# gaspardol/MonteCarloPredictiveCoding

Hardware: AMD Instinct MI355X
Metric: Langevin inference steps/sec (whole node), MNIST MCPC 784-256-256-30, batch 6000 (higher is better)
Workload: dtype f32

## Files before the change

### include/mcpc.h

```cpp
#ifndef MCPC_H
#define MCPC_H

#include <stdint.h>

#ifdef __cplusplus
extern "C" {
#endif

#define MCPC_ABI_VERSION 4
#define MCPC_MAX_LATENT 6

#define MCPC_OK 0
#define MCPC_EINVAL (-1)
#define MCPC_EHIP (-2)
#define MCPC_ENOMEM (-3)
#define MCPC_ESTATE (-4)

#define MCPC_ACT_IDENTITY 0
#define MCPC_ACT_RELU 1
#define MCPC_ACT_TANH 2

#define MCPC_LOSS_NONE 0
#define MCPC_LOSS_GAUSSIAN 1
#define MCPC_LOSS_BERNOULLI 2
// ... 66 lines not shown
const char* mcpc_last_error(void);
int mcpc_create(const mcpc_net_desc* desc, mcpc_engine** out);
int mcpc_destroy(mcpc_engine* e);

int mcpc_bind_params(mcpc_engine* e, int j, const float* W, const float* bias);
int mcpc_params_changed(mcpc_engine* e, void* stream);

int mcpc_bind_inputs(mcpc_engine* e, const float* inputs, void* stream);
int mcpc_bind_target(mcpc_engine* e, const float* target, void* stream);

int mcpc_load_state(mcpc_engine* e, const float* const* x, void* stream);
int mcpc_store_state(mcpc_engine* e, float* const* x, void* stream);

int mcpc_store_adam_state(mcpc_engine* e, float* const* m, float* const* v, void* stream);

int mcpc_run(mcpc_engine* e, const mcpc_run_desc* run, void* stream);

int mcpc_read_param_grads(mcpc_engine* e, int j, float* dW, float* db, float scale, int accumulate, void* stream);
int mcpc_read_param_grads_flat(mcpc_engine* e, float* flat, int64_t n_floats, float scale, void* stream);
int64_t mcpc_param_count(const mcpc_engine* e);

#define MCPC_COMM_ID_BYTES 128
int mcpc_comm_unique_id(void* id_out);
int mcpc_comm_init(mcpc_engine* e, int n_ranks, int rank, const void* id);
int mcpc_allreduce_grads(mcpc_engine* e, float* flat, int64_t n_floats, void* stream);
int mcpc_comm_destroy(mcpc_engine* e);

int mcpc_philox_normals(int device, uint64_t seed, uint64_t step, int layer, uint64_t chain_base,
                        int batch, int n_units, float* out, int raw, void* stream);

#define MCPC_MOM_IDENTITY 0
#define MCPC_MOM_SIGMOID  1

int mcpc_moments_accumulate(int device, const float* rec, int64_t row_elems, int32_t first, int32_t stride, int32_t n,
                            int32_t transform, double* sum, double* sumsq, int accumulate, void* stream);

int mcpc_sync_check(mcpc_engine* e, void* stream);

int mcpc_query(const mcpc_engine* e, int32_t* lds_bytes, int32_t* chains_per_wg, int32_t* n_workgroups,
               int32_t* spill_slots);
const char* mcpc_step_kernel_name(const mcpc_engine* e);
const char* mcpc_last_step_kernel_name(const mcpc_engine* e);
const char* mcpc_last_flush_plan(const mcpc_engine* e, int j);

int mcpc_set_profiling(mcpc_engine* e, int enable);
int mcpc_last_step_kernel_ms(mcpc_engine* e, float* ms, int32_t* n_launches, int64_t* n_steps);
int mcpc_last_shader_clock_ghz(mcpc_engine* e, float* ghz);

int mcpc_debug_poison_lds(int device, uint32_t word, void* stream);

int mcpc_debug_lw_jobs(int32_t n_latent, const int32_t* sizes, int32_t n_out, int32_t* fwd, int32_t* bwd, int32_t cap,
                       int32_t* n_fwd, int32_t* n_bwd, int32_t* tile);

#ifdef __cplusplus
}
#endif
#endif
```

### montecarlopredictivecoding_amd/_lib.py

```python
import ctypes as C
import os

MAX_LATENT = 6
COMM_ID_BYTES = 128
ENERGY_COLS = MAX_LATENT + 2
ABI_VERSION = 4

ACT_IDENTITY, ACT_RELU, ACT_TANH = 0, 1, 2
LOSS_NONE, LOSS_GAUSSIAN, LOSS_BERNOULLI = 0, 1, 2
XOPT_SGD, XOPT_ADAM = 0, 1
NOISE_NONE, NOISE_PHILOX, NOISE_EXTERNAL = 0, 1, 2
ENERGY_NONE, ENERGY_LAST, ENERGY_ALL = 0, 1, 2
MOM_IDENTITY, MOM_SIGMOID = 0, 1

LIB_PATH = os.environ.get("MCPC_LIB") or os.path.join(os.path.dirname(os.path.abspath(__file__)), "libmcpc.so")


class MCPCLibraryError(RuntimeError):
    pass


class MCPCError(RuntimeError):

    def __init__(self, code, message):
# ... 25 lines not shown
        ("beta1", C.c_double), ("beta2", C.c_double), ("eps", C.c_double),
        ("update_x", C.c_int32),
        ("noise_mode", C.c_int32), ("noise_var", C.c_double),
        ("seed", C.c_uint64), ("step_base", C.c_uint64), ("chain_base", C.c_uint64),
        ("ext_noise", C.c_void_p * MAX_LATENT),
        ("acc_begin", C.c_int32), ("acc_end", C.c_int32), ("acc_reset", C.c_int32),
        ("energy_mode", C.c_int32),
        ("energies_out", C.c_void_p),
        ("rec_begin", C.c_int32), ("rec_stride", C.c_int32), ("rec_count", C.c_int32),
        ("rec_x", C.c_void_p * MAX_LATENT),
        ("rec_out", C.c_void_p),
        ("xgrad", C.c_void_p * MAX_LATENT),
    ]


SYMBOLS = {
    "mcpc_abi_version": (C.c_int, []),
    "mcpc_build_info": (C.c_char_p, []),
    "mcpc_last_error": (C.c_char_p, []),
    "mcpc_create": (C.c_int, [C.POINTER(NetDesc), C.POINTER(C.c_void_p)]),
    "mcpc_destroy": (C.c_int, [C.c_void_p]),
    "mcpc_bind_params": (C.c_int, [C.c_void_p, C.c_int, C.c_void_p, C.c_void_p]),
    "mcpc_params_changed": (C.c_int, [C.c_void_p, C.c_void_p]),
    "mcpc_bind_inputs": (C.c_int, [C.c_void_p, C.c_void_p, C.c_void_p]),
    "mcpc_bind_target": (C.c_int, [C.c_void_p, C.c_void_p, C.c_void_p]),
    "mcpc_load_state": (C.c_int, [C.c_void_p, C.POINTER(C.c_void_p), C.c_void_p]),
    "mcpc_store_state": (C.c_int, [C.c_void_p, C.POINTER(C.c_void_p), C.c_void_p]),
    "mcpc_store_adam_state": (C.c_int, [C.c_void_p, C.POINTER(C.c_void_p), C.POINTER(C.c_void_p), C.c_void_p]),
    "mcpc_run": (C.c_int, [C.c_void_p, C.POINTER(RunDesc), C.c_void_p]),
    "mcpc_read_param_grads": (C.c_int, [C.c_void_p, C.c_int, C.c_void_p, C.c_void_p, C.c_float, C.c_int, C.c_void_p]),
    "mcpc_read_param_grads_flat": (C.c_int, [C.c_void_p, C.c_void_p, C.c_int64, C.c_float, C.c_void_p]),
    "mcpc_param_count": (C.c_int64, [C.c_void_p]),
    "mcpc_comm_unique_id": (C.c_int, [C.c_void_p]),
    "mcpc_comm_init": (C.c_int, [C.c_void_p, C.c_int, C.c_int, C.c_void_p]),
    "mcpc_allreduce_grads": (C.c_int, [C.c_void_p, C.c_void_p, C.c_int64, C.c_void_p]),
    "mcpc_comm_destroy": (C.c_int, [C.c_void_p]),
    "mcpc_philox_normals": (C.c_int, [C.c_int, C.c_uint64, C.c_uint64, C.c_int, C.c_uint64, C.c_int, C.c_int,
                                      C.c_void_p, C.c_int, C.c_void_p]),
    "mcpc_moments_accumulate": (C.c_int, [C.c_int, C.c_void_p, C.c_int64, C.c_int32, C.c_int32, C.c_int32, C.c_int32,
                                          C.c_void_p, C.c_void_p, C.c_int, C.c_void_p]),
    "mcpc_query": (C.c_int, [C.c_void_p, C.POINTER(C.c_int32), C.POINTER(C.c_int32), C.POINTER(C.c_int32),
                             C.POINTER(C.c_int32)]),
    "mcpc_step_kernel_name": (C.c_char_p, [C.c_void_p]),
    "mcpc_last_step_kernel_name": (C.c_char_p, [C.c_void_p]),
    "mcpc_last_flush_plan": (C.c_char_p, [C.c_void_p, C.c_int]),
    "mcpc_sync_check": (C.c_int, [C.c_void_p, C.c_void_p]),
    "mcpc_set_profiling": (C.c_int, [C.c_void_p, C.c_int]),
    "mcpc_last_step_kernel_ms": (C.c_int, [C.c_void_p, C.POINTER(C.c_float), C.POINTER(C.c_int32),
                                           C.POINTER(C.c_int64)]),
    "mcpc_last_shader_clock_ghz": (C.c_int, [C.c_void_p, C.POINTER(C.c_float)]),
    "mcpc_debug_poison_lds": (C.c_int, [C.c_int, C.c_uint32, C.c_void_p]),
    "mcpc_debug_lw_jobs": (C.c_int, [C.c_int32, C.POINTER(C.c_int32), C.c_int32, C.POINTER(C.c_int32), C.POINTER(C.c_int32), C.c_int32,
                                     C.POINTER(C.c_int32), C.POINTER(C.c_int32), C.POINTER(C.c_int32)]),
}

_lib = None


def load():
    global _lib
    if _lib is not None:
        return _lib
    if not os.path.exists(LIB_PATH):
        raise MCPCLibraryError(
            f"{LIB_PATH} not found: build it with `python -c 'import __graft_entry__ as g; g.build()'` "
            f"or `make -C montecarlopredictivecoding_amd/csrc`. There is no fallback path.")
    import torch
    try:
        lib = C.CDLL(LIB_PATH)
    except OSError as exc:
        raise MCPCLibraryError(f"could not load {LIB_PATH}: {exc}") from exc
    for name, (res, args) in SYMBOLS.items():
        try:
            fn = getattr(lib, name)
        except AttributeError as exc:
            raise MCPCLibraryError(f"{LIB_PATH} does not export {name}") from exc
        fn.restype = res
        fn.argtypes = args
    v = lib.mcpc_abi_version()
    if v != ABI_VERSION:
        raise MCPCLibraryError(f"libmcpc ABI {v} != binding ABI {ABI_VERSION}: rebuild the library")
    info = parse_build_info(lib.mcpc_build_info().decode("utf-8", "replace"))
    if info.get("exp") != "0" and os.environ.get("MCPC_ALLOW_EXP") != "1":
        raise MCPCLibraryError(f"{LIB_PATH} is a timing-experiment build ({info.get('flags')}): it computes wrong results on purpose. "
                               "Set MCPC_ALLOW_EXP=1 to load it for a timing A/B; unset MCPC_LIB to load the product.")
    _lib = lib
    return lib


def parse_build_info(line: str) -> dict:
    head, _, flags = line.partition(" flags=[")
    out = {"flags": flags[:-1] if flags.endswith("]") else flags}
    for word in head.split()[1:]:
        key, _, val = word.partition("=")
        out[key] = val
    return out


def build_info() -> dict:
    info = parse_build_info(load().mcpc_build_info().decode("utf-8", "replace"))
    info["path"] = LIB_PATH
    return info


def csrc_sha(root=None) -> str:
    import glob
# ... 15 lines not shown
```

### montecarlopredictivecoding_amd/csrc/mcpc_api.hip

```cpp
#include <hip/hip_runtime.h>
#include <dlfcn.h>
#include <rccl/rccl.h>

#include <algorithm>
#include <cmath>
#include <cstdarg>
#include <cstdio>
#include <cstdlib>
#include <cstring>
#include <string>
#include <vector>

#include "mcpc_build.h"
#include "mcpc_kernels.h"
#include "mcpc_moments.h"

using namespace mcpc;

namespace {

thread_local std::string g_err;

int fail(int code, const char* fmt, ...) {
    char buf[1024];
// ... 4 lines not shown
    g_err = buf;
    return code;
}

#define HIP_TRY(expr)                                                                            \
    do {                                                                                         \
        hipError_t _e = (expr);                                                                  \
        if (_e != hipSuccess) return fail(MCPC_EHIP, "%s failed: %s (%s:%d)", #expr, hipGetErrorString(_e), __FILE__, __LINE__); \
    } while (0)

inline int pad16(int n) { return (n + 15) / 16 * 16; }
inline int kblocks(int k_pad) { return (k_pad + kKB - 1) / kKB; }
inline int grid_for(size_t n, int block = 256) { return (int)std::min<size_t>((n + block - 1) / block, 4096); }
inline bool heb_wide(int et, int at) { return et >= 8 && at % 8 == 0 && (at <= 16 || at % 16 == 0); }
inline bool heb_narrow_in(int et, int at) { return !heb_wide(et, at) && et == 16 && (at == 1 || at == 2 || at == 4); }

struct Lin {
    const float* W = nullptr;
    const float* bias = nullptr;
    bool bound = false;
    int n_out = 0, n_in = 0, out_pad = 0, in_pad = 0;
    float* Wf = nullptr;
    float* Wb = nullptr;
    float* bias_pad = nullptr;
    float* G = nullptr;
    float* Gb = nullptr;
    int g_ld = 0;
    bool spill_tm = false;
    size_t slab_off = 0;
    size_t slab_floats = 0;
};

constexpr int kMaxRingParts = 8;
struct Knobs {
    int ws = -1;
    int wide = 0;
    int no_overlap = 0;
    int slot_cap = 384;
    int spill_gb = 0;
    int cu_slack = 0;
    int flush_streams = 2;
    int flush_tail = 0;
    int ring_parts = 3;
    int dw_ksplit = 0;
    int ws_prio = 0;
    int stagger = 0;
    int no_lean = 0;
    int no_ybits = 0;
    int overlay16 = 0;
    int no_xl = 0;
    int rr = 1;
    int rr_qmax = 100;
    int heb171 = 0;
    int heb_fp32 = 0;
    int u_row = 5000;
    int u_gemm0 = 1200;
    int u_kb = 200;
    int u_kbt = 68;
    int u_eh = 3000, u_eb = 1300, u_ef = 500;
};

int parse_tuning(const char* str, Knobs& k) {
    if (!str) return 0;
    std::string s(str);
    size_t pos = 0;
    while (pos < s.size()) {
        size_t end = s.find_first_of(",;", pos);
        if (end == std::string::npos) end = s.size();
        std::string item = s.substr(pos, end - pos);
        pos = end + 1;
        while (!item.empty() && item.front() == ' ') item.erase(item.begin());
        while (!item.empty() && item.back() == ' ') item.pop_back();
        if (item.empty()) continue;
        const size_t eq = item.find('=');
        const std::string key = item.substr(0, eq);
        const int val = eq == std::string::npos ? 1 : atoi(item.c_str() + eq + 1);
        struct { const char* name; int* dst; } table[] = {
            {"ws", &k.ws}, {"wide", &k.wide}, {"no_overlap", &k.no_overlap},
            {"slot_cap", &k.slot_cap}, {"spill_gb", &k.spill_gb}, {"cu_slack", &k.cu_slack}, {"ring_parts", &k.ring_parts}, {"flush_tail", &k.flush_tail}, {"flush_streams", &k.flush_streams}, {"dw_ksplit", &k.dw_ksplit},
            {"ws_prio", &k.ws_prio}, {"stagger", &k.stagger}, {"no_lean", &k.no_lean}, {"no_ybits", &k.no_ybits}, {"overlay16", &k.overlay16}, {"heb_fp32", &k.heb_fp32}, {"heb171", &k.heb171}, {"rr", &k.rr}, {"rr_qmax", &k.rr_qmax}, {"no_xl", &k.no_xl},
            {"u_row", &k.u_row}, {"u_gemm0", &k.u_gemm0}, {"u_kb", &k.u_kb}, {"u_kbt", &k.u_kbt}, {"u_eh", &k.u_eh}, {"u_eb", &k.u_eb}, {"u_ef", &k.u_ef}};
        bool found = false;
        for (auto& t : table)
            if (key == t.name) { *t.dst = val; found = true; }
        if (!found) return fail(MCPC_EINVAL, "unknown tuning key '%s' in mcpc_net_desc::tuning", key.c_str());
    }
    if (k.ws != -1 && k.ws != 0 && k.ws != 2 && k.ws != 3 && k.ws != 4)
        return fail(MCPC_EINVAL, "tuning ws=%d: 0 (barrier kernel), 2 (in-place kernel), 3 (unified-wave kernel) or 4 (layer-wise kernels)", k.ws);
    if (k.ws == 4) {
        const Knobs dflt;
        const struct { const char* name; bool set; } lds_only[] = {
            {"no_lean", k.no_lean != 0}, {"no_xl", k.no_xl != 0}, {"overlay16", k.overlay16 != 0}, {"rr", k.rr != dflt.rr},
            {"u_row", k.u_row != dflt.u_row}, {"u_gemm0", k.u_gemm0 != dflt.u_gemm0}, {"u_kb", k.u_kb != dflt.u_kb}, {"u_kbt", k.u_kbt != dflt.u_kbt},
            {"u_eh", k.u_eh != dflt.u_eh}, {"u_eb", k.u_eb != dflt.u_eb}, {"u_ef", k.u_ef != dflt.u_ef}};
        for (auto& t : lds_only)
            if (t.set) return fail(MCPC_EINVAL, "tuning ws=4 (layer-wise kernels) together with %s, a knob of the LDS-resident kernels", t.name);
    }
    if (k.slot_cap < 2) k.slot_cap = 2;
    if (k.cu_slack < 0) k.cu_slack = 0;
    if (k.ring_parts < 2 || k.ring_parts > kMaxRingParts) return fail(MCPC_EINVAL, "tuning ring_parts=%d: 2..%d", k.ring_parts, kMaxRingParts);
    return 0;
}

}

static const char* const kLwName = "mcpc::mcpc_lw_fwd_kernel + mcpc::mcpc_lw_bwd_kernel";

struct UPlan {
    bool ok = false;
    bool on = false;
    bool prefer = false;
    int lds_a[kMaxLatent]{}, lds_e[kMaxLatent]{}, lds_eo = 0, lds_red = 0, lds_ws_sync = 0, lds_zero = 0, lds_spillmax = 0, lds_rowexp = 0;
    int lds_x[kMaxLatent]{}, lds_bias[kMaxLatent]{}, lds_hbias = 0, lds_yw = 0, lds_bytes = 0;
    KPhase* phases = nullptr;
    int n_phases = 0;
};

struct mcpc_engine {
    mcpc_net_desc d{};
    Knobs knobs;
    ncclComm_t comm = nullptr;
    int comm_ranks = 0;
    int L = 0, Bpad = 0, nwg = 0, has_head = 0;
    int nwg_live = 0;
    static constexpr int ct = 16;
    int nw = kWaves;
    int ws = 0;
    int ws2_chunk = 0, ws2_ring = 0;
    bool ws2_overlay = true;
    int lds_ws_sync = 0;
    int npad[kMaxLatent]{};
    int out_pad = 0;
    Lin lin[kMaxLatent + 1];
    float* x[kMaxLatent]{};
    float* m[kMaxLatent]{};
    float* v[kMaxLatent]{};
    float* e0sum = nullptr;
    float* mu1 = nullptr;
    float* ypad = nullptr;
    float* ytile = nullptr;
    uint32_t* ybits = nullptr;
    int* y_binary = nullptr;
    int ywords = 0;
    bool target_bound = false;
    const float* inputs = nullptr;
    int slots = 0, half_slots = 0;
    hipStream_t aux = nullptr;
    hipEvent_t ev_steps[kMaxRingParts] = {}, ev_flush[kMaxRingParts] = {};
    hipStream_t spacer = nullptr;
    hipStream_t aux3 = nullptr;
// ... 1105 lines not shown
    const int nlin = e->L + (e->has_head ? 1 : 0);
    const int max_rows = e->half_slots * e->Bpad;
    size_t total = 0;
    for (int j = 1; j < nlin; ++j) {
        Lin& ln = e->lin[j];
        const HebPlan h = plan_hebbian(e, ln.out_pad, ln.in_pad, max_rows);
        ln.slab_off = total;
        ln.slab_floats = (size_t)h.ksplit_cap * ((size_t)ln.out_pad * ln.in_pad + ln.out_pad);
        total += ln.slab_floats;
    }
    if (!e->slab && (rc = dmalloc(e->slab, total))) return rc;
    e->slab_floats = total;
    e->spill_ready = true;
    return 0;
}

static inline int spill_id_a_host(int l) { return l; }
int flush_spill(mcpc_engine* e, int n_slots, int slot0, hipStream_t stream, int part) {
    const unsigned* const smax = e->spillmax + (size_t)part * kSpillTensors;
    const int rows = n_slots * e->Bpad;
    const int nlin = e->L + (e->has_head ? 1 : 0);
    ReduceJobs jobs{};
    unsigned max_blocks = 1;
    hipStream_t const main_stream = stream;
    const bool two = e->aux3 != nullptr && stream == e->aux;
    double load[2] = {0.0, 0.0};
    if (two) { HIP_TRY(hipEventRecord(e->ev_fork, main_stream)); HIP_TRY(hipStreamWaitEvent(e->aux3, e->ev_fork, 0)); }
    auto next_stream = [&](double cost) {
        const int k = (two && load[1] < load[0]) ? 1 : 0;
        load[k] += cost;
        return k ? e->aux3 : main_stream;
    };
    for (int j = 1; j < nlin; ++j) {
        Lin& ln = e->lin[j];
        const int ne = ln.out_pad, na = ln.in_pad;
        const float* E = (j < e->L ? e->spill_e[j] : e->spill_eo) + (size_t)slot0 * e->Bpad * ne;
        const float* A = e->spill_a[j - 1] + (size_t)slot0 * e->Bpad * na;
        const HebPlan h = plan_hebbian(e, ne, na, rows);
        std::string plan;
        auto name_launch = [&](const char* kern, int te, int ra, bool sw, int n_mt, int n_nt) {
            char buf[64];
            snprintf(buf, sizeof buf, "%s%s<%d,%d%s>x%d", plan.empty() ? "" : "+", kern, te, ra, sw ? ",T" : "", n_mt);
            plan += buf;
            if (n_nt > 1) plan += "*" + std::to_string(n_nt);
        };
        const char* const heb_name = e->knobs.heb_fp32 ? "heb" : "heb7";
        const int e_id = j < e->L ? kMaxLatent + j : kSpillIdEo;
        float* slab = e->slab + ln.slab_off;
        float* slab_b = slab + (size_t)h.ksplit * ne * na;
        if ((size_t)h.ksplit * ((size_t)ne * na + ne) > ln.slab_floats)
            return fail(MCPC_ESTATE, "internal: Hebbian slabs of Linear %d (%d splits) exceed their allocation", j, h.ksplit);
        if (h.swapped) {
            stream = next_stream((double)ne * na);
            HebArgs a{A, E, slab, slab_b, rows, na, ne, h.rps, 1, 1, h.ksplit, 0, smax + spill_id_a_host(j - 1), smax + e_id};
            name_launch(heb_name, h.te[0], 2, true, 1, 1);
            int rc = 0;
            if (!e->knobs.heb_fp32) {
                if (h.te[0] == 1) rc = launch_heb7<1, 2, true>(a, stream);
                else if (h.te[0] == 2) rc = launch_heb7<2, 2, true>(a, stream);
                else rc = launch_heb7<4, 2, true>(a, stream);
            } else
            if (h.te[0] == 1) rc = launch_heb<1, 2, true>(a, stream);
            else if (h.te[0] == 2) rc = launch_heb<2, 2, true>(a, stream);
            else rc = launch_heb<4, 2, true>(a, stream);
            if (rc) return rc;
        } else if (h.tiled) {
            int col = 0;
            for (int part = 0; part < 2; ++part) {
                if (h.n_mt[part] == 0) continue;
                HebArgs a{E, A, slab, slab_b, rows, ne, na, h.rps, h.n_mt[part], h.n_nt, h.ksplit, col, smax + e_id, smax + spill_id_a_host(j - 1)};
                stream = next_stream((double)h.n_mt[part] * h.te[part] * 16 * na);
                int rc = 0;
                const int te = h.te[part];
                const bool resplit = te == 17 && h.ra == 2 && !e->knobs.heb_fp32 && e->knobs.heb171;
                if (!resplit) name_launch(heb_name, te, h.ra, false, h.n_mt[part], h.n_nt);
                if (!e->knobs.heb_fp32) {
                    if (te == 17 && h.ra == 2 && !e->knobs.heb171) rc = launch_heb7<17, 2>(a, stream);
                    else if (te == 17 && h.ra == 2) {
                        HebArgs a1 = a;
                        a1.n_nt = 2 * a.n_nt;
                        name_launch(heb_name, 17, 1, false, a1.n_mt, a1.n_nt);
                        rc = launch_heb7<17, 1>(a1, stream);
                    }
                    else if (te == 16 && h.ra == 2) rc = launch_heb7<16, 2>(a, stream);
                    else if (te == 8 && h.ra == 2) rc = launch_heb7<8, 2>(a, stream);
                    else if (te == 17) rc = launch_heb7<17, 1>(a, stream);
                    else if (te == 16) rc = launch_heb7<16, 1>(a, stream);
                    else rc = launch_heb7<8, 1>(a, stream);
                } else
                if (te == 17 && h.ra == 2) rc = launch_heb<17, 2>(a, stream);
                else if (te == 16 && h.ra == 2) rc = launch_heb<16, 2>(a, stream);
                else if (te == 8 && h.ra == 2) rc = launch_heb<8, 2>(a, stream);
                else if (te == 17) rc = launch_heb<17, 1>(a, stream);
                else if (te == 16) rc = launch_heb<16, 1>(a, stream);
                else rc = launch_heb<8, 1>(a, stream);
                if (rc) return rc;
                col += h.n_mt[part] * te * 16;
            }
        } else {
            stream = next_stream((double)ne * na);
            hipLaunchKernelGGL(mcpc_dw_kernel, dim3((h.wave_tiles + 3) / 4, h.ksplit), dim3(256), 0, stream, E, A, slab, slab_b,
                               rows, ne, na, h.rps);
            plan = "dw tiles=" + std::to_string(h.wave_tiles);
        }
        e->last_flush[j] = plan + " ksplit=" + std::to_string(h.ksplit) + " rps=" + std::to_string(h.rps) + (ln.spill_tm ? " tm" : " rm");
        const float sign = j < e->L ? -1.0f : 1.0f;
        jobs.job[jobs.n_jobs++] = ReduceJob{slab, ln.G, ne * na, h.ksplit, sign, h.swapped ? ne : 0, h.swapped ? na : 0};
        jobs.job[jobs.n_jobs++] = ReduceJob{slab_b, ln.Gb, ne, h.ksplit, sign, 0, 0};
        max_blocks = std::max(max_blocks, (unsigned)std::min<size_t>(((size_t)ne * na + 255) / 256, 2048));
    }
    stream = main_stream;
    if (two) { HIP_TRY(hipEventRecord(e->ev_join, e->aux3)); HIP_TRY(hipStreamWaitEvent(main_stream, e->ev_join, 0)); }
    if (jobs.n_jobs > 0)
        hipLaunchKernelGGL(mcpc_reduce_jobs_kernel, dim3(max_blocks, jobs.n_jobs), dim3(256), 0, stream, jobs);
    HIP_TRY(hipGetLastError());
    return 0;
}

}

extern "C" {

int mcpc_run(mcpc_engine* e, const mcpc_run_desc* r, void* stream_) {
// ... 566 lines not shown
    __syncthreads();
    if (poison_lds[(threadIdx.x * 97) % (160 * 1024 / 4)] != word) atomicAdd(&seen[8 * 256], 1);
}
}
extern "C" {

int mcpc_debug_poison_lds(int device, uint32_t word, void* stream_) {
    HIP_TRY(hipSetDevice(device));
    int n_cu = 256;
    if (hipDeviceGetAttribute(&n_cu, hipDeviceAttributeMultiprocessorCount, device) != hipSuccess || n_cu <= 0) n_cu = 256;
    static bool attr_set[16] = {false};
    if (device >= 0 && device < 16 && !attr_set[device]) {
        HIP_TRY(hipFuncSetAttribute((const void*)mcpc_poison_lds_kernel, hipFuncAttributeMaxDynamicSharedMemorySize, 160 * 1024));
        attr_set[device] = true;
    }
    int* seen = nullptr;
    HIP_TRY(hipMalloc((void**)&seen, (8 * 256 + 1) * sizeof(int)));
    hipStream_t stream = (hipStream_t)stream_;
    int rc = MCPC_OK;
    for (int pass = 0; pass < 2 && rc == MCPC_OK; ++pass) {
        if (hipMemsetAsync(seen, 0, (8 * 256 + 1) * sizeof(int), stream) != hipSuccess) { rc = fail(MCPC_EHIP, "hipMemsetAsync failed"); break; }
        hipLaunchKernelGGL(mcpc_poison_lds_kernel, dim3(4 * n_cu), dim3(256), 160 * 1024, stream, word, seen);
        if (hipGetLastError() != hipSuccess || hipStreamSynchronize(stream) != hipSuccess) rc = fail(MCPC_EHIP, "the LDS poison kernel failed");
    }
    if (rc == MCPC_OK) {
        std::vector<int> h(8 * 256 + 1);
        if (hipMemcpy(h.data(), seen, h.size() * sizeof(int), hipMemcpyDeviceToHost) != hipSuccess) rc = fail(MCPC_EHIP, "hipMemcpy failed");
        else {
            int visited = 0;
            for (int i = 0; i < 8 * 256; ++i) visited += h[i] > 0;
            if (visited < n_cu) rc = fail(MCPC_ESTATE, "LDS poison reached %d of %d compute units", visited, n_cu);
            else if (h[8 * 256] != 0) rc = fail(MCPC_ESTATE, "LDS poison read-back mismatch");
        }
    }
    (void)hipFree(seen);
    return rc;
}

int mcpc_debug_lw_jobs(int32_t n_latent, const int32_t* sizes, int32_t n_out, int32_t* fwd, int32_t* bwd, int32_t cap,
                       int32_t* n_fwd, int32_t* n_bwd, int32_t* tile) {
    if (n_latent < 1 || n_latent > kMaxLatent || !sizes || n_out < 0) return fail(MCPC_EINVAL, "bad network");
    int npad[kMaxLatent];
    for (int l = 0; l < n_latent; ++l) { if (sizes[l] < 1) return fail(MCPC_EINVAL, "sizes[%d]=%d", l, sizes[l]); npad[l] = pad16(sizes[l]); }
    std::vector<LwJob> f, b;
    lw_job_table(n_latent, npad, pad16(n_out), f, b);
    for (int i = 0; i < (int)f.size() && i < cap && fwd; ++i) { fwd[2 * i] = f[i].layer; fwd[2 * i + 1] = f[i].ut0; }
    for (int i = 0; i < (int)b.size() && i < cap && bwd; ++i) { bwd[2 * i] = b[i].layer; bwd[2 * i + 1] = b[i].ut0; }
    if (n_fwd) *n_fwd = (int32_t)f.size();
    if (n_bwd) *n_bwd = (int32_t)b.size();
    if (tile) { tile[0] = kLwChains; tile[1] = kLwUnitTiles; }
    return MCPC_OK;
}

int mcpc_set_profiling(mcpc_engine* e, int enable) {
    if (!e) return fail(MCPC_EINVAL, "null engine");
    HIP_TRY(hipSetDevice(e->d.device));
    e->profiling = enable != 0;
    e->events_used = 0;
    e->prof_steps = 0;
    if (enable) HIP_TRY(hipMemset(e->clk, 0, 2 * sizeof(unsigned long long)));
    return MCPC_OK;
}

namespace {
int sum_events(const std::vector<std::pair<hipEvent_t, hipEvent_t>>& ev, size_t used, float* total) {
    *total = 0.f;
    for (size_t i = 0; i < used; ++i) {
        HIP_TRY(hipEventSynchronize(ev[i].second));
        float t = 0.f;
        HIP_TRY(hipEventElapsedTime(&t, ev[i].first, ev[i].second));
        *total += t;
    }
    return 0;
}
}

int mcpc_last_step_kernel_ms(mcpc_engine* e, float* ms, int32_t* n_launches, int64_t* n_steps) {
    if (!e || !ms) return fail(MCPC_EINVAL, "null argument");
    HIP_TRY(hipSetDevice(e->d.device));
    const int rc = sum_events(e->events, e->events_used, ms);
    if (rc) return rc;
    if (n_launches) *n_launches = (int32_t)e->events_used;
    if (n_steps) *n_steps = (int64_t)std::llround(e->prof_steps);
    return MCPC_OK;
}

}
```

### montecarlopredictivecoding_amd/csrc/mcpc_hebbian.h

```cpp
#pragma once

namespace mcpc {

constexpr int kHebKB = 32;
constexpr int kHebThreads = 512;

struct HebArgs {
    const float* E;
    const float* A;
    float* slab;
    float* slab_b;
    int rows, ne, na;
    int rows_per_split;
    int n_mt, n_nt, ksplit;
    int e_col_base;
    const unsigned* e_max;
    const unsigned* a_max;
};

#ifndef MCPC_HEB_LD_AUX
#define MCPC_HEB_LD_AUX 0
#endif
#ifndef MCPC_HEB_LDS_PAD
#define MCPC_HEB_LDS_PAD 16
#endif
constexpr int heb_lds_stride(int row_floats) { return row_floats == 256 ? row_floats + MCPC_HEB_LDS_PAD : row_floats; }

__device__ __forceinline__ void heb_glds16(const float* gsrc, float* lds_dst) {
    __builtin_amdgcn_global_load_lds((const __attribute__((address_space(1))) void*)gsrc,
                                     (__attribute__((address_space(3))) void*)lds_dst, 16, 0, MCPC_HEB_LD_AUX);
}

template <int TE, int RA, bool SWAPPED = false>
__global__ __launch_bounds__(kHebThreads, 2) void mcpc_heb_kernel(const HebArgs P) {
    constexpr int TA = 8 * RA;
    constexpr int LDE = 16 * TE, LDA = 16 * TA;
    constexpr int LDE_S = heb_lds_stride(LDE), LDA_S = heb_lds_stride(LDA);
    constexpr int E_PIECES = kHebKB * LDE / 256;
    constexpr int A_PIECES = kHebKB * LDA / 256;
    constexpr int PIECES = E_PIECES + A_PIECES;
    constexpr int PPW = (PIECES + 7) / 8;
    constexpr int STAGE = kHebKB * (LDE_S + LDA_S);
    static_assert(kHebKB * LDE % 256 == 0 && kHebKB * LDA % 256 == 0, "panels must be whole 1 KiB pieces");
    extern __shared__ __attribute__((aligned(16))) float lds[];

    const int tid = threadIdx.x, lane = tid & 63;
    const int w = __builtin_amdgcn_readfirstlane(tid >> 6);
    const int m = lane & 15, kq = lane >> 4;

    const int total = P.n_mt * P.n_nt * P.ksplit;
    int id = blockIdx.x;
    if (total % 8 == 0) id = (id & 7) * (total >> 3) + (id >> 3);
    const int per_split = P.n_mt * P.n_nt;
    const int split = id / per_split, rem = id - split * per_split;
    const int nt = rem / P.n_mt, mt = rem - nt * P.n_mt;
    const int e_col0 = P.e_col_base + mt * LDE, a_col0 = nt * LDA;
    const int r0 = split * P.rows_per_split;
    const int r1 = min(P.rows, r0 + P.rows_per_split);
    const int n_stage = (r1 - r0) / kHebKB;

    for (int i = tid; i < 2 * STAGE / 4; i += kHebThreads) reinterpret_cast<f32x4*>(lds)[i] = splat(0.f);
    __syncthreads();

    int g_off[PPW], l_off[PPW];
    bool p_on[PPW], p_is_a[PPW];
#pragma unroll
    for (int k = 0; k < PPW; ++k) {
        const int p = w + 8 * k;
        const bool is_a = p >= E_PIECES;
        const int c = (is_a ? p - E_PIECES : p) * 64 + lane;
// ... 37 lines not shown
        do {                                                                                    \
            _Pragma("unroll") for (int i = 0; i < TE; ++i) e_[i] = Ep[(ks_) * 4 * LDE_S + 16 * i]; \
            _Pragma("unroll") for (int j = 0; j < RA; ++j) a_[j] = Ap[(ks_) * 4 * LDA_S + 16 * j]; \
        } while (0)
#define HEB_MFMA(e_, a_)                                                                        \
        do {                                                                                    \
            _Pragma("unroll") for (int i = 0; i < TE; ++i)                                      \
                _Pragma("unroll") for (int j = 0; j < RA; ++j) acc[i][j] = mfma16(e_[i], a_[j], acc[i][j]); \
        } while (0)
        HEB_LOAD(eA, aA, 0);
#pragma unroll
        for (int ks = 0; ks < kHebKB / 4; ks += 2) {
            __builtin_amdgcn_sched_barrier(0);
            HEB_LOAD(eB, aB, ks + 1);
            HEB_MFMA(eA, aA);
            __builtin_amdgcn_sched_barrier(0);
            if (ks + 2 < kHebKB / 4) HEB_LOAD(eA, aA, ks + 2);
            HEB_MFMA(eB, aB);
        }
        __builtin_amdgcn_sched_barrier(0);
#undef HEB_LOAD
#undef HEB_MFMA
        if (does_bias) {
            const float* col = lds + buf * STAGE + (SWAPPED ? kHebKB * LDE_S : 0) + tid;
#pragma unroll 8
            for (int r = 0; r < kHebKB; ++r) bsum += col[r * (SWAPPED ? LDA_S : LDE_S)];
        }
        __syncthreads();
    }

    float* out = P.slab + (size_t)split * P.ne * P.na;
#pragma unroll
    for (int i = 0; i < TE; ++i) {
        const int u0 = e_col0 + 16 * i + 4 * kq;
        if (u0 >= P.ne) continue;
#pragma unroll
        for (int j = 0; j < RA; ++j) {
            const int a = a_col0 + 16 * (RA * w + j) + m;
            if (a >= P.na) continue;
#pragma unroll
            for (int reg = 0; reg < 4; ++reg) out[(size_t)(u0 + reg) * P.na + a] = acc[i][j][reg];
        }
    }
    if constexpr (SWAPPED) {
        if (does_bias && a_col0 + tid < P.na) P.slab_b[(size_t)split * P.na + a_col0 + tid] = bsum;
    } else {
        if (does_bias && e_col0 + tid < P.ne) P.slab_b[(size_t)split * P.ne + e_col0 + tid] = bsum;
    }
}

constexpr int kHeb7KB = 32;
constexpr int kHeb7LD = 40;

template <int TE, int RA, bool SWAPPED = false>
__global__ __launch_bounds__(kHebThreads, 2) void mcpc_heb7_kernel(const HebArgs P) {
    constexpr int TPW = (TE + 7) / 8;
    constexpr int PLANE = 16 * TE * kHeb7LD;
    constexpr int NPL = 2;
    extern __shared__ __attribute__((aligned(16))) unsigned short lds7[];
    const int tid = threadIdx.x, lane = tid & 63;
    const int w = __builtin_amdgcn_readfirstlane(tid >> 6);
    const int m = lane & 15, g = lane >> 4;
    const int c = lane & 15, q = lane >> 4;
    const int total = P.n_mt * P.n_nt * P.ksplit;
    int id = blockIdx.x;
    if (total % 8 == 0) id = (id & 7) * (total >> 3) + (id >> 3);
    const int per_split = P.n_mt * P.n_nt;
    const int split = id / per_split, rem = id - split * per_split;
    const int nt = rem / P.n_mt, mt = rem - nt * P.n_mt;
    const int e_col0 = P.e_col_base + mt * 16 * TE, a_col0 = nt * 16 * 8 * RA;
    const int net = P.ne / 16, nat = P.na / 16;
    const int e_tile0 = e_col0 / 16, a_tile0 = a_col0 / 16 + RA * w;
    const int r0 = split * P.rows_per_split;
    const int r1 = min(P.rows, r0 + P.rows_per_split);
    const int n_stage = (r1 - r0) / kHeb7KB;
    const size_t rt_base = (size_t)r0 / 16;
    const int e_exp = scale_exp_for_max(__uint_as_float(*P.e_max)), a_exp = scale_exp_for_max(__uint_as_float(*P.a_max));
    const float e_scale = pow2i(e_exp), a_scale = pow2i(a_exp);

    typedef const char __attribute__((address_space(1)))* gb_t;
    bool e_on[TPW];
#pragma unroll
    for (int i = 0; i < TPW; ++i) e_on[i] = (w + 8 * i) < TE && e_tile0 + w + 8 * i < net;
    bool a_on[RA];
#pragma unroll
    for (int j = 0; j < RA; ++j) a_on[j] = a_tile0 + j < nat;
    const uint32_t e_lane = 16u * (uint32_t)lane;
    const size_t e_rt_bytes = (size_t)net * 1024, a_rt_bytes = (size_t)nat * 1024;
    f32x4 eraw[TPW][2];
    f32x4 araw[RA][2];
    float* const a_scr = reinterpret_cast<float*>(lds7 + 2 * NPL * PLANE) + 16 * TE + (size_t)w * (2 * 272);
    const int a_wr = 4 * (17 * q + c);
    const int a_rd = 4 * (17 * (m >> 2) + 4 * g) + (m & 3);
    const int s_last = n_stage > 0 ? n_stage - 1 : 0;
    auto load_e = [&](int s_) {
#if defined(MCPC_HEB_EXP) && MCPC_HEB_EXP == 4
        if (P.rows >= 0) return;
#endif
        const int s = s_ < s_last ? s_ : s_last;
        const gb_t base = (gb_t)P.E + (rt_base + 2 * (size_t)s) * e_rt_bytes;
#pragma unroll
        for (int i = 0; i < TPW; ++i) {
            const gb_t tb = base + (size_t)(e_on[i] ? e_tile0 + w + 8 * i : e_tile0) * 1024;
#pragma unroll
            for (int b = 0; b < 2; ++b) {
                eraw[i][b] = __builtin_nontemporal_load(reinterpret_cast<const gf32x4*>(tb + b * e_rt_bytes + e_lane));
            }
        }
    };
    auto load_a = [&](int s_) {
#if defined(MCPC_HEB_EXP) && MCPC_HEB_EXP == 4
        if (P.rows >= 0) return;
#endif
        const int s = s_ < s_last ? s_ : s_last;
        const gb_t base = (gb_t)P.A + (rt_base + 2 * (size_t)s) * a_rt_bytes;
#pragma unroll
        for (int j = 0; j < RA; ++j) {
            const gb_t tb = base + (size_t)(a_on[j] ? a_tile0 + j : 0) * 1024;
#pragma unroll
            for (int b = 0; b < 2; ++b)
                araw[j][b] = __builtin_nontemporal_load(reinterpret_cast<const gf32x4*>(tb + b * a_rt_bytes + e_lane));
        }
    };
    float* const bias_lds = reinterpret_cast<float*>(lds7 + 2 * NPL * PLANE);
    float asum[RA];
#pragma unroll
    for (int j = 0; j < RA; ++j) asum[j] = 0.f;
    const bool e_bias = !SWAPPED && nt == 0, a_bias = SWAPPED && mt == 0;

    auto split_store = [&](int buf, bool real) {
#if defined(MCPC_HEB_EXP) && MCPC_HEB_EXP == 2
        if (P.rows >= 0) return;
#endif
        unsigned short* const base = lds7 + (size_t)buf * NPL * PLANE + (size_t)(4 * q) * kHeb7LD + 2 * c;
#pragma unroll
        for (int i = 0; i < TPW; ++i) {
            if ((w + 8 * i) >= TE) continue;
            const f32x4 v0 = e_on[i] ? eraw[i][0] : splat(0.f), v1 = e_on[i] ? eraw[i][1] : splat(0.f);
            if (e_bias && real) {
                f32x4 t = v0 + v1;
#pragma unroll
                for (int u = 0; u < 4; ++u) {
                    float v = t[u];
                    v += __shfl_xor(v, 1, 64); v += __shfl_xor(v, 2, 64); v += __shfl_xor(v, 4, 64); v += __shfl_xor(v, 8, 64);
                    t[u] = v;
                }
                if (c == 0) {
                    f32x4* const bp = reinterpret_cast<f32x4*>(bias_lds + 16 * (w + 8 * i) + 4 * q);
                    *bp = *bp + t;
                }
            }
#pragma unroll
            for (int u = 0; u < 4; ++u) {
                unsigned h, mm;
                split2_pair(f32x2{v0[u], v1[u]}, e_scale, h, mm);
                unsigned short* const dst = base + (size_t)(16 * (w + 8 * i) + u) * kHeb7LD;
                *reinterpret_cast<unsigned*>(dst) = h;
                *reinterpret_cast<unsigned*>(dst + PLANE) = mm;
            }
        }
    };
    struct Op { u32x4 h, m; };
    auto make_a = [&](int j) {
#pragma unroll
        for (int b = 0; b < 2; ++b) *reinterpret_cast<f32x4*>(a_scr + b * 272 + a_wr) = a_on[j] ? araw[j][b] : splat(0.f);
        __builtin_amdgcn_fence(__ATOMIC_RELEASE, "wavefront");
        __builtin_amdgcn_wave_barrier();
        __builtin_amdgcn_fence(__ATOMIC_ACQUIRE, "wavefront");
        Op o;
#pragma unroll
        for (int i = 0; i < 4; ++i) {
            unsigned h, mm;
            const float a0 = a_scr[a_rd + 4 * i], a1 = a_scr[272 + a_rd + 4 * i];
            split2_pair(f32x2{a0, a1}, a_scale, h, mm);
            o.h[i] = h; o.m[i] = mm;
            if (a_bias) asum[j] += a0 + a1;
        }
        __builtin_amdgcn_fence(__ATOMIC_RELEASE, "wavefront");
        __builtin_amdgcn_wave_barrier();
        return o;
    };

    f32x4 acc[TE][RA];
#pragma unroll
    for (int i = 0; i < TE; ++i)
#pragma unroll
        for (int j = 0; j < RA; ++j) acc[i][j] = splat(0.f);

    auto mfma_stage = [&](int buf, const Op (&ao)[RA]) {
#if defined(MCPC_HEB_EXP) && MCPC_HEB_EXP == 5
        if (P.rows >= 0) return;
#endif
        const unsigned short* const rd = lds7 + (size_t)buf * NPL * PLANE + (size_t)m * kHeb7LD + 8 * g;
        u32x4 eh = *reinterpret_cast<const u32x4*>(rd), em = *reinterpret_cast<const u32x4*>(rd + PLANE);
#pragma unroll
        for (int i = 0; i < TE; ++i) {
            const unsigned short* const nx = rd + (size_t)(16 * (i + 1 < TE ? i + 1 : i)) * kHeb7LD;
            __builtin_amdgcn_sched_barrier(0);
            const u32x4 ehn = *reinterpret_cast<const u32x4*>(nx), emn = *reinterpret_cast<const u32x4*>(nx + PLANE);
#define H7(e_, ap_) _Pragma("unroll") for (int j = 0; j < RA; ++j) acc[i][j] = mfma4(e_, ao[j].ap_, acc[i][j])
            H7(em, h); H7(eh, m); H7(eh, h);
#undef H7
            __builtin_amdgcn_sched_barrier(0);
            eh = ehn; em = emn;
        }
    };

    if (tid < 16 * TE) bias_lds[tid] = 0.f;
    __syncthreads();
    if (n_stage == 0) return;
    load_e(0);
    load_a(0);
    split_store(0, true);
    load_e(1);
    __syncthreads();
#if defined(MCPC_HEB_EXP) && MCPC_HEB_EXP == 3
    if (w < 8) {
#else
    if (w < 4) {
#endif
        for (int s = 0; s < n_stage; ++s) {
            split_store((s + 1) & 1, s + 1 < n_stage);
            load_e(s + 2);
            Op ao[RA];
#pragma unroll
            for (int j = 0; j < RA; ++j) ao[j] = make_a(j);
            load_a(s + 1);
            mfma_stage(s & 1, ao);
            __syncthreads();
        }
    } else {
        for (int s = 0; s < n_stage; ++s) {
            Op ao[RA];
#pragma unroll
            for (int j = 0; j < RA; ++j) ao[j] = make_a(j);
            load_a(s + 1);
            mfma_stage(s & 1, ao);
            split_store((s + 1) & 1, s + 1 < n_stage);
            load_e(s + 2);
            __syncthreads();
        }
    }

    const float unscale = pow2i(-e_exp) * pow2i(-a_exp);
    float* out = P.slab + (size_t)split * P.ne * P.na;
#pragma unroll
    for (int i = 0; i < TE; ++i) {
        const int u0 = e_col0 + 16 * i + 4 * g;
        if (u0 >= P.ne) continue;
#pragma unroll
        for (int j = 0; j < RA; ++j) {
            const int a = a_col0 + 16 * (RA * w + j) + m;
            if (a >= P.na) continue;
#pragma unroll
            for (int reg = 0; reg < 4; ++reg) out[(size_t)(u0 + reg) * P.na + a] = acc[i][j][reg] * unscale;
        }
    }
    if (e_bias) {
#pragma unroll
        for (int i = 0; i < TPW; ++i) {
            if ((w + 8 * i) >= TE || !e_on[i]) continue;
            if (c == 0) *reinterpret_cast<f32x4*>(P.slab_b + (size_t)split * P.ne + 16 * (e_tile0 + w + 8 * i) + 4 * q) =
                            *reinterpret_cast<const f32x4*>(bias_lds + 16 * (w + 8 * i) + 4 * q);
        }
    }
    if (a_bias) {
#pragma unroll
        for (int j = 0; j < RA; ++j) {
            float v = asum[j];
            v += __shfl_xor(v, 16, 64); v += __shfl_xor(v, 32, 64);
            if (g == 0 && a_on[j]) P.slab_b[(size_t)split * P.na + 16 * (a_tile0 + j) + m] = v;
        }
    }
}

struct ReduceJob {
    const float* slab;
    float* dst;
    int n, ksplit;
    float sign;
    int tr_cols, tr_ld;
};
constexpr int kMaxReduceJobs = 2 * (kMaxLatent + 1);
struct ReduceJobs {
    ReduceJob job[kMaxReduceJobs];
    int n_jobs;
};

__global__ __launch_bounds__(256) void mcpc_reduce_jobs_kernel(const ReduceJobs J) {
    __shared__ float part[4][64];
    const ReduceJob jb = J.job[blockIdx.y];
    const size_t n = (size_t)jb.n;
// ... 35 lines not shown
```

Baseline: 17750.

## Add software L2 prefetch touches to Hebbian kernel and restructure TE=17 loads

Adds per-thread 'touch' loads in the Hebbian dW kernel that read one word per cache line of future E/A row tiles, a configurable distance (heb_pf, default 0) ahead, to warm the cache before the real nontemporal loads. It also splits the 17th E tile across two waves with narrow f32x2 loads instead of a third full tile slot, zeroes the padding rows in LDS, and raises the occupancy hint for small TE. A debug API exposes the touch address map. The extra loads add memory traffic and register pressure in exchange for hiding load latency.

```diff
diff --git a/include/mcpc.h b/include/mcpc.h
--- a/include/mcpc.h
+++ b/include/mcpc.h
@@ -142,6 +142,10 @@
 int mcpc_debug_lw_jobs(int32_t n_latent, const int32_t* sizes, int32_t n_out, int32_t* fwd, int32_t* bwd, int32_t cap,
                        int32_t* n_fwd, int32_t* n_bwd, int32_t* tile);
 
+int mcpc_debug_heb_touch_map(int32_t te, int32_t ra, int32_t swapped, int32_t ne, int32_t na, int32_t rows, int32_t rows_per_split,
+                             int32_t n_mt, int32_t n_nt, int32_t e_col_base, int32_t block, int32_t stage, int32_t pf,
+                             int64_t* off, int32_t* kind, int32_t cap, int32_t* n, int32_t* stages);
+
 #ifdef __cplusplus
 }
 #endif
diff --git a/montecarlopredictivecoding_amd/_lib.py b/montecarlopredictivecoding_amd/_lib.py
--- a/montecarlopredictivecoding_amd/_lib.py
+++ b/montecarlopredictivecoding_amd/_lib.py
@@ -101,6 +101,8 @@
     "mcpc_debug_poison_lds": (C.c_int, [C.c_int, C.c_uint32, C.c_void_p]),
     "mcpc_debug_lw_jobs": (C.c_int, [C.c_int32, C.POINTER(C.c_int32), C.c_int32, C.POINTER(C.c_int32), C.POINTER(C.c_int32), C.c_int32,
                                      C.POINTER(C.c_int32), C.POINTER(C.c_int32), C.POINTER(C.c_int32)]),
+    "mcpc_debug_heb_touch_map": (C.c_int, [C.c_int32] * 13 + [C.POINTER(C.c_int64), C.POINTER(C.c_int32), C.c_int32, C.POINTER(C.c_int32),
+                                           C.POINTER(C.c_int32)]),
 }
 
 _lib = None
diff --git a/montecarlopredictivecoding_amd/csrc/mcpc_api.hip b/montecarlopredictivecoding_amd/csrc/mcpc_api.hip
--- a/montecarlopredictivecoding_amd/csrc/mcpc_api.hip
+++ b/montecarlopredictivecoding_amd/csrc/mcpc_api.hip
@@ -80,6 +80,7 @@
     int rr = 1;
     int rr_qmax = 100;
     int heb171 = 0;
+    int heb_pf = 0;
     int heb_fp32 = 0;
     int u_row = 5000;
     int u_gemm0 = 1200;
@@ -106,7 +107,7 @@
         struct { const char* name; int* dst; } table[] = {
             {"ws", &k.ws}, {"wide", &k.wide}, {"no_overlap", &k.no_overlap},
             {"slot_cap", &k.slot_cap}, {"spill_gb", &k.spill_gb}, {"cu_slack", &k.cu_slack}, {"ring_parts", &k.ring_parts}, {"flush_tail", &k.flush_tail}, {"flush_streams", &k.flush_streams}, {"dw_ksplit", &k.dw_ksplit},
-            {"ws_prio", &k.ws_prio}, {"stagger", &k.stagger}, {"no_lean", &k.no_lean}, {"no_ybits", &k.no_ybits}, {"overlay16", &k.overlay16}, {"heb_fp32", &k.heb_fp32}, {"heb171", &k.heb171}, {"rr", &k.rr}, {"rr_qmax", &k.rr_qmax}, {"no_xl", &k.no_xl},
+            {"ws_prio", &k.ws_prio}, {"stagger", &k.stagger}, {"no_lean", &k.no_lean}, {"no_ybits", &k.no_ybits}, {"overlay16", &k.overlay16}, {"heb_fp32", &k.heb_fp32}, {"heb171", &k.heb171}, {"heb_pf", &k.heb_pf}, {"rr", &k.rr}, {"rr_qmax", &k.rr_qmax}, {"no_xl", &k.no_xl},
             {"u_row", &k.u_row}, {"u_gemm0", &k.u_gemm0}, {"u_kb", &k.u_kb}, {"u_kbt", &k.u_kbt}, {"u_eh", &k.u_eh}, {"u_eb", &k.u_eb}, {"u_ef", &k.u_ef}};
         bool found = false;
         for (auto& t : table)
@@ -124,6 +125,7 @@
         for (auto& t : lds_only)
             if (t.set) return fail(MCPC_EINVAL, "tuning ws=4 (layer-wise kernels) together with %s, a knob of the LDS-resident kernels", t.name);
     }
+    if (k.heb_pf < 0 || k.heb_pf > kHebMaxPf) return fail(MCPC_EINVAL, "tuning heb_pf=%d: 0..%d", k.heb_pf, kHebMaxPf);
     if (k.slot_cap < 2) k.slot_cap = 2;
     if (k.cu_slack < 0) k.cu_slack = 0;
     if (k.ring_parts < 2 || k.ring_parts > kMaxRingParts) return fail(MCPC_EINVAL, "tuning ring_parts=%d: 2..%d", k.ring_parts, kMaxRingParts);
@@ -1335,7 +1337,7 @@
             return fail(MCPC_ESTATE, "internal: Hebbian slabs of Linear %d (%d splits) exceed their allocation", j, h.ksplit);
         if (h.swapped) {
             stream = next_stream((double)ne * na);
-            HebArgs a{A, E, slab, slab_b, rows, na, ne, h.rps, 1, 1, h.ksplit, 0, smax + spill_id_a_host(j - 1), smax + e_id};
+            HebArgs a{A, E, slab, slab_b, rows, na, ne, h.rps, 1, 1, h.ksplit, 0, smax + spill_id_a_host(j - 1), smax + e_id, e->knobs.heb_pf};
             name_launch(heb_name, h.te[0], 2, true, 1, 1);
             int rc = 0;
             if (!e->knobs.heb_fp32) {
@@ -1351,7 +1353,7 @@
             int col = 0;
             for (int part = 0; part < 2; ++part) {
                 if (h.n_mt[part] == 0) continue;
-                HebArgs a{E, A, slab, slab_b, rows, ne, na, h.rps, h.n_mt[part], h.n_nt, h.ksplit, col, smax + e_id, smax + spill_id_a_host(j - 1)};
+                HebArgs a{E, A, slab, slab_b, rows, ne, na, h.rps, h.n_mt[part], h.n_nt, h.ksplit, col, smax + e_id, smax + spill_id_a_host(j - 1), e->knobs.heb_pf};
                 stream = next_stream((double)h.n_mt[part] * h.te[part] * 16 * na);
                 int rc = 0;
                 const int te = h.te[part];
@@ -2024,6 +2026,46 @@
     return MCPC_OK;
 }
 
+int mcpc_debug_heb_touch_map(int32_t te, int32_t ra, int32_t swapped, int32_t ne, int32_t na, int32_t rows, int32_t rows_per_split,
+                             int32_t n_mt, int32_t n_nt, int32_t e_col_base, int32_t block, int32_t stage, int32_t pf,
+                             int64_t* off, int32_t* kind, int32_t cap, int32_t* n, int32_t* stages) {
+    static const int inst[][3] = {{8, 1, 0}, {8, 2, 0}, {16, 1, 0}, {16, 2, 0}, {17, 1, 0}, {17, 2, 0}, {1, 2, 1}, {2, 2, 1}, {4, 2, 1}};
+    bool known = false;
+    for (auto& i : inst) known = known || (i[0] == te && i[1] == ra && i[2] == (swapped != 0));
+    if (!known) return fail(MCPC_EINVAL, "no mcpc_heb7_kernel<%d, %d, %s>", te, ra, swapped ? "true" : "false");
+    if (ne < 16 || na < 16 || ne % 16 || na % 16 || rows < 32 || rows % 32 || rows_per_split < 32 || rows_per_split % 32 || n_mt < 1 || n_nt < 1 ||
+        e_col_base < 0 || e_col_base % 16 || pf < 0 || pf > kHebMaxPf)
+        return fail(MCPC_EINVAL, "bad Hebbian launch");
+    const int ksplit = (rows + rows_per_split - 1) / rows_per_split;
+    const int total = n_mt * n_nt * ksplit;
+    if (block < 0 || block >= total) return fail(MCPC_EINVAL, "block %d of %d", block, total);
+    int id = block;
+    if (total % 8 == 0) id = (id & 7) * (total >> 3) + (id >> 3);
+    const int per_split = n_mt * n_nt;
+    const int split = id / per_split, rem = id - split * per_split;
+    const int nt = rem / n_mt, mt = rem - nt * n_mt;
+    const int e_tile0 = (e_col_base + mt * 16 * te) / 16, a_tile0 = nt * 8 * ra;
+    const int net = ne / 16, nat = na / 16;
+    const int r0 = split * rows_per_split, r1 = std::min(rows, r0 + rows_per_split);
+    const int n_stage = (r1 - r0) / kHeb7KB;
+    if (stage < -pf || stage >= n_stage) return fail(MCPC_EINVAL, "iteration %d of a split of %d stages (the prologue runs -pf .. -1)", stage, n_stage);
+    const int s_last = n_stage - 1;
+    const int64_t rt_base = r0 / 16;
+    const int count = heb_touch_on(te, ra) ? heb_touch_slots(te, ra) * kHebThreads : 0;
+    if (n) *n = count;
+    if (stages) {
+        stages[0] = heb_touch_stage(stage, false, pf, s_last); stages[1] = heb_touch_stage(stage, true, pf, s_last);
+        stages[2] = n_stage; stages[3] = (int32_t)rt_base; stages[4] = e_tile0; stages[5] = a_tile0;
+    }
+    for (int L = 0; L < count && L < cap && off && kind; ++L) {
+        const HebTouch t = heb_touch_line(te, ra, L, e_tile0, a_tile0, net, nat);
+        const int64_t rt = rt_base + 2 * (int64_t)heb_touch_stage(stage, t.is_a, pf, s_last);
+        off[L] = rt * (t.is_a ? nat : net) * 1024 + t.off;
+        kind[L] = (t.is_a ? 1 : 0) | (t.filler ? 2 : 0);
+    }
+    return MCPC_OK;
+}
+
 int mcpc_set_profiling(mcpc_engine* e, int enable) {
     if (!e) return fail(MCPC_EINVAL, "null engine");
     HIP_TRY(hipSetDevice(e->d.device));
diff --git a/montecarlopredictivecoding_amd/csrc/mcpc_hebbian.h b/montecarlopredictivecoding_amd/csrc/mcpc_hebbian.h
--- a/montecarlopredictivecoding_amd/csrc/mcpc_hebbian.h
+++ b/montecarlopredictivecoding_amd/csrc/mcpc_hebbian.h
@@ -16,6 +16,7 @@
     int e_col_base;
     const unsigned* e_max;
     const unsigned* a_max;
+    int pf;
 };
 
 #ifndef MCPC_HEB_LD_AUX
@@ -159,9 +160,34 @@
 constexpr int kHeb7KB = 32;
 constexpr int kHeb7LD = 40;
 
+constexpr int kHebMaxPf = 4;
+constexpr bool heb_touch_on(int te, int ra) { return !(te == 17 && ra == 2); }
+constexpr int heb_touch_slots(int te, int ra) { return (16 * (te + 8 * ra) + kHebThreads - 1) / kHebThreads; }
+struct HebTouch {
+    bool is_a, filler;
+    unsigned off;
+};
+__host__ __device__ inline bool heb_touch_is_a(int ra, int L) { return L < 128 * ra; }
+__host__ __device__ inline HebTouch heb_touch_line(int te, int ra, int L, int e_tile0, int a_tile0, int net, int nat) {
+    HebTouch t;
+    t.is_a = heb_touch_is_a(ra, L);
+    const int k = t.is_a ? L : L - 128 * ra;
+    const int tile = k >> 4, b = (k >> 3) & 1, line = k & 7;
+    const int first = t.is_a ? a_tile0 : e_tile0, ntile = t.is_a ? nat : net;
+    t.filler = !((t.is_a || tile < te) && first + tile < ntile);
+    t.off = t.filler ? (unsigned)first * 1024u : (unsigned)(first + tile) * 1024u + (unsigned)b * ((unsigned)ntile * 1024u) + (unsigned)line * 128u;
+    return t;
+}
+__host__ __device__ inline int heb_touch_stage(int s, bool is_a, int pf, int s_last) {
+    const int st = s + (is_a ? 1 : 2) + pf;
+    return st < s_last ? st : s_last;
+}
+
 template <int TE, int RA, bool SWAPPED = false>
-__global__ __launch_bounds__(kHebThreads, 2) void mcpc_heb7_kernel(const HebArgs P) {
+__global__ __launch_bounds__(kHebThreads, (TE <= 4 ? 4 : 2)) void mcpc_heb7_kernel(const HebArgs P) {
     constexpr int TPW = (TE + 7) / 8;
+    constexpr bool X17 = TE == 17;
+    constexpr int TPWF = X17 ? 2 : TPW;
     constexpr int PLANE = 16 * TE * kHeb7LD;
     constexpr int NPL = 2;
     extern __shared__ __attribute__((aligned(16))) unsigned short lds7[];
@@ -194,11 +220,14 @@
     for (int j = 0; j < RA; ++j) a_on[j] = a_tile0 + j < nat;
     const uint32_t e_lane = 16u * (uint32_t)lane;
     const size_t e_rt_bytes = (size_t)net * 1024, a_rt_bytes = (size_t)nat * 1024;
-    f32x4 eraw[TPW][2];
+    f32x4 eraw[TPWF][2];
+    f32x2 xraw[2];
+    const int x_half = w == 0 ? 0 : 1;
+    const bool x_on = X17 && (w == 0 || w == 5) && e_tile0 + 16 < net;
     f32x4 araw[RA][2];
     float* const a_scr = reinterpret_cast<float*>(lds7 + 2 * NPL * PLANE) + 16 * TE + (size_t)w * (2 * 272);
-    const int a_wr = 4 * (17 * q + c);
-    const int a_rd = 4 * (17 * (m >> 2) + 4 * g) + (m & 3);
+    int a_wr = 4 * (17 * q + c);
+    int a_rd = 4 * (17 * (m >> 2) + 4 * g) + (m & 3);
     const int s_last = n_stage > 0 ? n_stage - 1 : 0;
     auto load_e = [&](int s_) {
 #if defined(MCPC_HEB_EXP) && MCPC_HEB_EXP == 4
@@ -207,13 +236,19 @@
         const int s = s_ < s_last ? s_ : s_last;
         const gb_t base = (gb_t)P.E + (rt_base + 2 * (size_t)s) * e_rt_bytes;
 #pragma unroll
-        for (int i = 0; i < TPW; ++i) {
+        for (int i = 0; i < TPWF; ++i) {
             const gb_t tb = base + (size_t)(e_on[i] ? e_tile0 + w + 8 * i : e_tile0) * 1024;
 #pragma unroll
             for (int b = 0; b < 2; ++b) {
                 eraw[i][b] = __builtin_nontemporal_load(reinterpret_cast<const gf32x4*>(tb + b * e_rt_bytes + e_lane));
             }
         }
+        if constexpr (X17) {
+            const gb_t tb = base + (size_t)(x_on ? e_tile0 + 16 : e_on[0] ? e_tile0 + w : e_tile0) * 1024 + 8 * x_half;
+#pragma unroll
+            for (int b = 0; b < 2; ++b)
+                xraw[b] = __builtin_nontemporal_load(reinterpret_cast<const __attribute__((address_space(1))) f32x2*>(tb + b * e_rt_bytes + e_lane));
+        }
     };
     auto load_a = [&](int s_) {
 #if defined(MCPC_HEB_EXP) && MCPC_HEB_EXP == 4
@@ -229,6 +264,31 @@
                 araw[j][b] = __builtin_nontemporal_load(reinterpret_cast<const gf32x4*>(tb + b * a_rt_bytes + e_lane));
         }
     };
+    constexpr int NTCH = heb_touch_slots(TE, RA);
+    uint32_t t_off[NTCH], t_val[NTCH];
+#pragma unroll
+    for (int k = 0; k < NTCH; ++k) {
+        t_off[k] = heb_touch_line(TE, RA, kHebThreads * k + tid, e_tile0, a_col0 / 16, net, nat).off;
+        t_val[k] = 0;
+    }
+    auto touch = [&](int s) {
+        if constexpr (!heb_touch_on(TE, RA)) return;
+#if defined(MCPC_HEB_EXP) && MCPC_HEB_EXP == 4
+        if (P.rows >= 0) return;
+#endif
+#pragma unroll
+        for (int k = 0; k < NTCH; ++k) {
+            const bool is_a = heb_touch_is_a(RA, kHebThreads * k + 64 * w);
+            const size_t rt = rt_base + 2 * (size_t)heb_touch_stage(s, is_a, P.pf, s_last);
+            const gb_t base = is_a ? (gb_t)P.A + rt * a_rt_bytes : (gb_t)P.E + rt * e_rt_bytes;
+            t_val[k] = *reinterpret_cast<const __attribute__((address_space(1))) uint32_t*>(base + t_off[k]);
+        }
+    };
+    auto touch_done = [&]() {
+        if constexpr (!heb_touch_on(TE, RA)) return;
+#pragma unroll
+        for (int k = 0; k < NTCH; ++k) asm volatile("" ::"v"(t_val[k]));
+    };
     float* const bias_lds = reinterpret_cast<float*>(lds7 + 2 * NPL * PLANE);
     float asum[RA];
 #pragma unroll
@@ -241,7 +301,7 @@
 #endif
         unsigned short* const base = lds7 + (size_t)buf * NPL * PLANE + (size_t)(4 * q) * kHeb7LD + 2 * c;
 #pragma unroll
-        for (int i = 0; i < TPW; ++i) {
+        for (int i = 0; i < TPWF; ++i) {
             if ((w + 8 * i) >= TE) continue;
             const f32x4 v0 = e_on[i] ? eraw[i][0] : splat(0.f), v1 = e_on[i] ? eraw[i][1] : splat(0.f);
             if (e_bias && real) {
@@ -266,6 +326,32 @@
                 *reinterpret_cast<unsigned*>(dst + PLANE) = mm;
             }
         }
+        if constexpr (X17) {
+            if (x_on) {
+                const f32x2 v0 = xraw[0], v1 = xraw[1];
+                if (e_bias && real) {
+                    f32x2 t = v0 + v1;
+#pragma unroll
+                    for (int u = 0; u < 2; ++u) {
+                        float v = t[u];
+                        v += __shfl_xor(v, 1, 64); v += __shfl_xor(v, 2, 64); v += __shfl_xor(v, 4, 64); v += __shfl_xor(v, 8, 64);
+                        t[u] = v;
+                    }
+                    if (c == 0) {
+                        f32x2* const bp = reinterpret_cast<f32x2*>(bias_lds + 16 * 16 + 4 * q + 2 * x_half);
+                        *bp = *bp + t;
+                    }
+                }
+#pragma unroll
+                for (int u = 0; u < 2; ++u) {
+                    unsigned h, mm;
+                    split2_pair(f32x2{v0[u], v1[u]}, e_scale, h, mm);
+                    unsigned short* const dst = base + (size_t)(16 * 16 + 2 * x_half + u) * kHeb7LD;
+                    *reinterpret_cast<unsigned*>(dst) = h;
+                    *reinterpret_cast<unsigned*>(dst + PLANE) = mm;
+                }
+            }
+        }
     };
     struct Op { u32x4 h, m; };
     auto make_a = [&](int j) {
@@ -314,13 +400,32 @@
     };
 
     if (tid < 16 * TE) bias_lds[tid] = 0.f;
+    if constexpr (X17) {
+        for (int i = tid; i < 2 * NPL * 16 * (kHeb7LD / 2); i += kHebThreads) {
+            const int row = i / (kHeb7LD / 2), d = i - row * (kHeb7LD / 2);
+            reinterpret_cast<unsigned*>(lds7 + (size_t)(row >> 4) * PLANE + (size_t)(16 * 16 + (row & 15)) * kHeb7LD)[d] = 0u;
+        }
+    }
     __syncthreads();
     if (n_stage == 0) return;
     load_e(0);
     load_a(0);
     split_store(0, true);
     load_e(1);
+    uint32_t t_pro[kHebMaxPf][NTCH];
+#pragma unroll
+    for (int d = 0; d < kHebMaxPf; ++d) {
+        touch(d < P.pf ? d - P.pf : -1);
+#pragma unroll
+        for (int k = 0; k < NTCH; ++k) t_pro[d][k] = t_val[k];
+    }
     __syncthreads();
+    if constexpr (heb_touch_on(TE, RA)) {
+#pragma unroll
+        for (int d = 0; d + 1 < kHebMaxPf; ++d)
+#pragma unroll
+            for (int k = 0; k < NTCH; ++k) asm volatile("" ::"v"(t_pro[d][k]));
+    }
 #if defined(MCPC_HEB_EXP) && MCPC_HEB_EXP == 3
     if (w < 8) {
 #else
@@ -333,10 +438,18 @@
 #pragma unroll
             for (int j = 0; j < RA; ++j) ao[j] = make_a(j);
             load_a(s + 1);
+            touch_done();
+            touch(s);
             mfma_stage(s & 1, ao);
             __syncthreads();
         }
     } else {
+        if constexpr (X17 && RA == 2) {
+            int l2 = lane;
+            asm volatile("" : "+v"(l2));
+            a_wr = 4 * (17 * (l2 >> 4) + (l2 & 15));
+            a_rd = 4 * (17 * ((l2 & 15) >> 2) + 4 * (l2 >> 4)) + (l2 & 3);
+        }
         for (int s = 0; s < n_stage; ++s) {
             Op ao[RA];
 #pragma unroll
@@ -345,6 +458,8 @@
             mfma_stage(s & 1, ao);
             split_store((s + 1) & 1, s + 1 < n_stage);
             load_e(s + 2);
+            touch_done();
+            touch(s);
             __syncthreads();
         }
     }
```

After: 16980. -4.3%, worse.
